# saninsteinn/django-assistant-bot

Measured on AMD Instinct MI355X. Metric: RAG queries/sec + p50 end-to-end latency, bge-base + Llama-3-8B, 1/2/4/8 MI355X, higher is better.
Workload: dtype bf16; 1 GPU; model=bge-base-en + llama-3-8b, global_batch=128, seq_len=1090, parallelism=dp1, mode=batch, index_rows=1000000, index=single shard, local top-k (no collective), sampling=temperature=1.0 top_k=50 top_p=0.95 ignore_eos, graphs=True

## Files before the change

django_assistant_bot_amd/build.py:

```python
from __future__ import annotations

import argparse
import concurrent.futures as cf
import os
import subprocess
import sys
import sysconfig
from pathlib import Path

PKG = Path(__file__).resolve().parent
CSRC = PKG / "csrc"
BUILD = PKG / "_build"
ARCH = os.environ.get("DAB_OFFLOAD_ARCH", "gfx950")


def _hipcc() -> str:
    rocm = os.environ.get("ROCM_PATH", "/opt/rocm")
    cand = Path(rocm) / "bin" / "hipcc"
    return str(cand) if cand.exists() else "hipcc"


def ext_path() -> Path:
    suffix = sysconfig.get_config_var("EXT_SUFFIX") or ".so"
    return PKG / f"_native{suffix}"
# ... 73 lines not shown
        raise RuntimeError(f"native build failed for: {failed}")
    if force or jobs_list or not out.exists():
        link = [hipcc, f"--offload-arch={ARCH}", "-shared", "-fPIC", *[str(o) for o in objs], "-o", str(out), "-lpthread", "-ldl"]
        cmd, rc, log = _compile(link)
        if rc:
            print(" ".join(cmd), file=sys.stderr)
            print(log, file=sys.stderr)
            raise RuntimeError("native link failed")
    return out


SANITIZERS = {"asan": ["-fsanitize=address,undefined", "-fno-omit-frame-pointer", "-fno-sanitize-recover=undefined"],
              "tsan": ["-fsanitize=thread"]}


def selftest(kind: str = "asan", out_dir: Path | None = None) -> tuple[int, str]:
    out_dir = out_dir or BUILD
    out_dir.mkdir(exist_ok=True)
    exe = out_dir / f"runtime_selftest_{kind}"
    srcs = [CSRC / "tests" / "runtime_selftest.cpp", *sorted((CSRC / "runtime").glob("*.cpp"))]
    cmd = ["g++", "-std=c++17", "-g", "-O1", *SANITIZERS[kind], f"-I{CSRC}", *map(str, srcs), "-o", str(exe),
           "-ldl", "-lpthread"]
    _, rc, log = _compile(cmd)
    if rc:
        return rc, log
    p = subprocess.run([str(exe)], stdout=subprocess.PIPE, stderr=subprocess.STDOUT, text=True, timeout=600)
    return p.returncode, p.stdout


def main() -> None:
    ap = argparse.ArgumentParser(description=__doc__)
    ap.add_argument("--force", action="store_true")
    ap.add_argument("-j", "--jobs", type=int, default=None)
    ap.add_argument("--debug", action="store_true")
    ap.add_argument("-v", "--verbose", action="store_true")
    ap.add_argument("--selftest", choices=sorted(SANITIZERS), default=None)
    a = ap.parse_args()
    if a.selftest:
        rc, log = selftest(a.selftest)
        print(log)
        sys.exit(rc)
    print(build(force=a.force, jobs=a.jobs, debug=a.debug, verbose=a.verbose))


if __name__ == "__main__":
    main()
```

django_assistant_bot_amd/csrc/bindings.cpp:

```cpp
#include <hip/hip_runtime.h>
#include <pybind11/numpy.h>
#include <pybind11/pybind11.h>
#include <pybind11/stl.h>

#include <stdexcept>
#include <string>

#include "kernels/launchers.h"
#include "runtime/json_grammar.h"
#include "runtime/kv_manager.h"
#include "runtime/rag.h"
#include "runtime/tokenizer.h"
#include "runtime/trace.h"

namespace py = pybind11;
using u = uintptr_t;

#define VP(x) reinterpret_cast<void*>(x)
#define CVP(x) reinterpret_cast<const void*>(x)
#define ST(x) reinterpret_cast<hipStream_t>(x)

static void check(int err, const char* name) {
  if (err) throw std::runtime_error(std::string("dab kernel '") + name + "' failed: " + hipGetErrorString((hipError_t)err));
}

PYBIND11_MODULE(_native, m) {
// ... 379 lines not shown
           [](dab::SchemaMatcher& j, int remaining, u out) {
             py::gil_scoped_release rel;
             return j.fill_mask(remaining, (uint32_t*)out);
           })
      .def("advance", &dab::SchemaMatcher::advance)
      .def("done", &dab::SchemaMatcher::done)
      .def("broken", &dab::SchemaMatcher::broken)
      .def("completion_len", &dab::SchemaMatcher::completion_len)
      .def("text", [](const dab::SchemaMatcher& j) { return py::bytes(j.text()); });
  m.def("json_accepts", [](const py::bytes& b, bool complete, int max_depth, int max_ws) {
    return dab::json_accepts(std::string(b), complete, max_depth, max_ws);
  }, py::arg("bytes"), py::arg("complete") = true, py::arg("max_depth") = 64, py::arg("max_ws") = 255);

  py::class_<dab::KVBlockManager>(m, "KVBlockManager")
      .def(py::init<int, int, bool>(), py::arg("num_blocks"), py::arg("block_size"), py::arg("prefix_cache") = true)
      .def("add_sequence", &dab::KVBlockManager::add_sequence)
      .def("extend", &dab::KVBlockManager::extend)
      .def("append_tokens", &dab::KVBlockManager::append_tokens)
      .def("commit_prefix", &dab::KVBlockManager::commit_prefix)
      .def("free_sequence", &dab::KVBlockManager::free_sequence)
      .def("has", &dab::KVBlockManager::has)
      .def("num_tokens", &dab::KVBlockManager::num_tokens)
      .def("capacity_tokens", &dab::KVBlockManager::capacity_tokens)
      .def("num_free_blocks", &dab::KVBlockManager::num_free_blocks)
      .def("num_blocks", &dab::KVBlockManager::num_blocks)
      .def("block_size", &dab::KVBlockManager::block_size)
      .def("prefix_hits", &dab::KVBlockManager::prefix_hits)
      .def("blocks", &dab::KVBlockManager::blocks)
      .def("slot_mapping_into",
           [](const dab::KVBlockManager& k, int64_t seq, int start, int n, u out) {
             k.slot_mapping(seq, start, n, (int64_t*)out);
// ... 36 lines not shown
```

django_assistant_bot_amd/csrc/runtime/kv_manager.cpp:

```cpp
#include "kv_manager.h"

#include <algorithm>
#include <functional>
#include <iterator>
#include <stdexcept>

namespace dab {

KVBlockManager::KVBlockManager(int num_blocks, int block_size, bool prefix_cache)
    : num_blocks_(num_blocks), block_size_(block_size), prefix_cache_(prefix_cache) {
  if (num_blocks <= 0 || block_size <= 0) throw std::invalid_argument("num_blocks and block_size must be > 0");
  free_.reserve(num_blocks);
  for (int b = 0; b < num_blocks; ++b) free_.push_back(b);
  lru_cap_ = std::max(64, num_blocks / 4);
  ref_.assign(num_blocks, 0);
  block_hash_.assign(num_blocks, 0);
  lru_pos_.resize(num_blocks);
  in_lru_.assign(num_blocks, 0);
}

uint64_t KVBlockManager::chain_hash(uint64_t parent, const int32_t* toks, int n) const {
  uint64_t h = parent ^ 0x9E3779B97F4A7C15ull;
  for (int i = 0; i < n; ++i) {
    h ^= (uint64_t)(uint32_t)toks[i] + 0x9E3779B97F4A7C15ull + (h << 6) + (h >> 2);
// ... 35 lines not shown
      block_hash_[e] = 0;
      push_free(e);
    }
  } else {
    block_hash_[b] = 0;
    push_free(b);
  }
}

void KVBlockManager::push_free(int32_t b) {
  free_.push_back(b);
  std::push_heap(free_.begin(), free_.end(), std::greater<int32_t>());
}

int KVBlockManager::add_sequence(int64_t seq_id, const std::vector<int32_t>& tokens, int reserve) {
  if (seqs_.count(seq_id)) throw std::invalid_argument("sequence already registered");
  const int n = (int)tokens.size();
  const int need_tokens = n + (reserve > 0 ? reserve : 0);
  const int need_blocks = (need_tokens + block_size_ - 1) / block_size_;
  std::vector<int32_t> hit_blocks;
  std::vector<uint64_t> hit_hashes;
  if (prefix_cache_ && n > 1) {
    const int max_full = (n - 1) / block_size_;
    uint64_t h = 0;
    for (int i = 0; i < max_full; ++i) {
      h = chain_hash(h, tokens.data() + (size_t)i * block_size_, block_size_);
      auto it = cached_.find(h);
      if (it == cached_.end()) break;
      hit_blocks.push_back(it->second);
      hit_hashes.push_back(h);
    }
  }
  int reused_from_lru = 0;
  for (int32_t b : hit_blocks) reused_from_lru += in_lru_[b] ? 1 : 0;
  const int fresh = need_blocks - (int)hit_blocks.size();
  if (fresh > num_free_blocks() - reused_from_lru) return -1;
  Seq s;
  for (int32_t b : hit_blocks) {
    if (in_lru_[b]) {
      lru_.erase(lru_pos_[b]);
      in_lru_[b] = 0;
    }
    ++ref_[b];
    s.blocks.push_back(b);
  }
  s.hashes = hit_hashes;
  for (int i = 0; i < fresh; ++i) s.blocks.push_back(alloc_block());
  s.tokens = tokens;
  const int cached_tokens = (int)hit_blocks.size() * block_size_;
  prefix_hits_ += cached_tokens;
  seqs_.emplace(seq_id, std::move(s));
  return cached_tokens;
}

bool KVBlockManager::extend(int64_t seq_id, int n) {
  auto it = seqs_.find(seq_id);
  if (it == seqs_.end()) throw std::invalid_argument("unknown sequence");
  Seq& s = it->second;
  const int need = (int)s.tokens.size() + n;
  const int need_blocks = (need + block_size_ - 1) / block_size_;
  const int more = need_blocks - (int)s.blocks.size();
  if (more <= 0) return true;
  if (more > num_free_blocks()) return false;
// ... 36 lines not shown

int KVBlockManager::num_tokens(int64_t seq_id) const {
  auto it = seqs_.find(seq_id);
  return it == seqs_.end() ? 0 : (int)it->second.tokens.size();
}

int KVBlockManager::capacity_tokens(int64_t seq_id) const {
  auto it = seqs_.find(seq_id);
  return it == seqs_.end() ? 0 : (int)it->second.blocks.size() * block_size_;
}

const std::vector<int32_t>& KVBlockManager::blocks(int64_t seq_id) const {
  auto it = seqs_.find(seq_id);
  if (it == seqs_.end()) throw std::invalid_argument("unknown sequence");
  return it->second.blocks;
}

void KVBlockManager::slot_mapping(int64_t seq_id, int start, int n, int64_t* out) const {
  const auto& bl = blocks(seq_id);
  for (int i = 0; i < n; ++i) {
    const int pos = start + i;
    const int bi = pos / block_size_;
    if (bi >= (int)bl.size()) throw std::out_of_range("slot beyond allocated blocks");
    out[i] = (int64_t)bl[bi] * block_size_ + (pos % block_size_);
  }
}

int KVBlockManager::prepare_decode(const std::vector<int64_t>& seq_ids, const std::vector<int32_t>& tokens,
                                   int max_blocks, int32_t* ids, int32_t* pos, int64_t* slots, int32_t* ctx,
                                   int32_t* block_table) {
// ... 34 lines not shown
```

django_assistant_bot_amd/csrc/runtime/kv_manager.h:

```cpp
#pragma once
#include <cstdint>
#include <list>
#include <unordered_map>
#include <vector>

namespace dab {

class KVBlockManager {
 public:
  KVBlockManager(int num_blocks, int block_size, bool prefix_cache);

  int add_sequence(int64_t seq_id, const std::vector<int32_t>& tokens, int reserve);
  bool extend(int64_t seq_id, int n);
  void append_tokens(int64_t seq_id, const std::vector<int32_t>& tokens);
  void commit_prefix(int64_t seq_id, int n_computed);
  void free_sequence(int64_t seq_id);

  bool has(int64_t seq_id) const { return seqs_.count(seq_id) != 0; }
  int num_tokens(int64_t seq_id) const;
  int capacity_tokens(int64_t seq_id) const;
  int num_free_blocks() const { return (int)free_.size() + (int)lru_.size(); }
  int num_blocks() const { return num_blocks_; }
  int block_size() const { return block_size_; }
  int64_t prefix_hits() const { return prefix_hits_; }
  const std::vector<int32_t>& blocks(int64_t seq_id) const;

  int prepare_decode(const std::vector<int64_t>& seq_ids, const std::vector<int32_t>& tokens, int max_blocks,
                     int32_t* ids, int32_t* pos, int64_t* slots, int32_t* ctx, int32_t* block_table);
  void slot_mapping(int64_t seq_id, int start, int n, int64_t* out) const;
  void block_table(const std::vector<int64_t>& seq_ids, int max_blocks, int32_t* out) const;

 private:
  struct Seq {
    std::vector<int32_t> blocks;
    std::vector<int32_t> tokens;
    std::vector<uint64_t> hashes;
  };
  int num_blocks_, block_size_;
  bool prefix_cache_;
  std::vector<int32_t> free_;
// ... 18 lines not shown
```

django_assistant_bot_amd/engine/llm_engine.py:

```python
from __future__ import annotations

import itertools
import math
import os
import time
from collections import deque
from dataclasses import dataclass, field

import numpy as np
import torch

from .. import ops
from ..models import AttnMeta, KVCache, LlamaModel, decoder_config, random_decoder_weights
from ..models.configs import DecoderConfig
from ..ops._lib import native
from ..utils import trace
from .tokenizer import Tokenizer


@dataclass
class SamplingParams:
    max_new_tokens: int = 1024
    temperature: float = 1.0
    top_k: int = 50
# ... 10 lines not shown

@dataclass
class GenerationOutput:
    request_id: int
    prompt_ids: list
    token_ids: list
    text: str
    finish_reason: str
    usage: dict
    timings: dict


@dataclass
class _Req:
    rid: int
    prompt: list
    params: SamplingParams
    arrival: float
    out: list = field(default_factory=list)
    computed: int = 0
    admitted: bool = False
    first_token_t: float = 0.0
    finish_t: float = 0.0
    finish_reason: str = ""
    rng_base: int = 0
    prefill_s: float = 0.0
    preempted: int = 0
    matcher: object = None

    @property
    def seq(self):
        return self.rid

    def full_prompt(self):
        return self.prompt + self.out if self.preempted else self.prompt




def _bucket_sizes(max_batch):
    b = [1, 2, 4, 8, 16, 24, 32, 48, 64, 96, 128, 160, 192, 224, 256, 320, 384, 448, 512]
    return [x for x in b if x < max_batch] + [max_batch]


class LLMEngine:
    def __init__(self, model: str | DecoderConfig = "llama-3-8b", device=None, weights: dict | None = None,
                 checkpoint: str | None = None, seed: int = 0, max_batch: int = 256, block_size: int = 64,
                 max_model_len: int | None = None, kv_cache_gb: float | None = None, num_blocks: int | None = None,
                 max_prefill_tokens: int = 16384, use_graphs: bool = True, prefix_cache: bool = True,
                 tp_group=None, tp_size: int = 1, tp_rank: int = 0, interleaved_mlp: bool = True,
                 part_size: int = 512, kv_memory_fraction: float = 0.85, mixed_prefill_tokens: int = 0,
                 pipeline_decode: bool = True, shared_model: LlamaModel | None = None,
                 kv_cache_dtype: str | None = None, kv_scratch_blocks: int | None = None,
                 weight_dtype: str | None = None):
        self.cfg = decoder_config(model) if isinstance(model, str) else model
        cfg = self.cfg
        if shared_model is not None:
            have = getattr(shared_model, "weight_dtype", "bf16")
            if weight_dtype is not None and weight_dtype != have:
                raise ValueError(f"weight_dtype={weight_dtype!r} conflicts with the shared model's {have!r}")
            weight_dtype = have
        elif weight_dtype is None:
            weight_dtype = os.environ.get("DAB_WEIGHT_DTYPE") or "bf16"
        if weight_dtype not in ("bf16", "fp8"):
            raise ValueError(f"weight_dtype must be 'bf16' or 'fp8', got {weight_dtype!r}")
        if weight_dtype == "fp8" and tp_size > 1:
            raise ValueError("weight_dtype='fp8' does not support tensor parallelism (tp_size > 1) yet")
        self.weight_dtype = weight_dtype
        if kv_cache_dtype is None:
# ... 100 lines not shown
        self._h_bt = mk((mb, self.max_blocks_per_seq), dtype=torch.int32)
        self._h_temp = mk(mb, dtype=torch.float32)
        self._h_topk = mk(mb, dtype=torch.int32)
        self._h_topp = mk(mb, dtype=torch.float32)
        self._h_cnt = mk(mb, dtype=torch.int64)
        self._h_tokens = mk(mb, dtype=torch.int32)
        self._h_order = mk(mb, dtype=torch.int32)
        self.pipeline_decode = bool(pipeline_decode) and tp_size == 1
        self._h_alt = {k: mk(*(getattr(self, k).shape,), dtype=getattr(self, k).dtype)
                       for k in ("_h_ids", "_h_pos", "_h_slots", "_h_ctx", "_h_bt", "_h_temp", "_h_topk", "_h_topp",
                                 "_h_cnt", "_h_tokens", "_h_order")}
        self._inflight = None
        self._d_mask = None
        self._masked = False
        self._pending_prefill = None
        max_parts = math.ceil(self.max_model_len / part_size)
        self._workspace = ops.DecodeWorkspace(mb, cfg.heads // tp_size, cfg.head_dim, max_parts, dev) if self.is_gpu \
            else None
        self._sample_ws = ops.kernels.sample_workspace(mb, cfg.vocab_size, dev) if self.is_gpu else None
        self.vp = bool(getattr(self.model, "vocab_parallel", False))
        self._vp_cand = None
        if self.vp and self.is_gpu:
            ncl = ops.kernels.sample_candidates_per_row(self.model.vocab_local)
            self._vp_cand = torch.zeros((2, mb, ncl), dtype=torch.int32, device=dev)
        self._graphs: dict = {}
        self._buckets = _bucket_sizes(max_batch)
        self._graph_pool = None
        self.timer = trace.GpuTimer(enabled=self.is_gpu)
        self.fault_hook = None
        self.auto_expire = True

    def add_request(self, prompt_ids: list, params: SamplingParams | None = None, request_id: int | None = None) -> int:
        params = params or SamplingParams()
        rid = next(self._ids) if request_id is None else request_id
        prompt = [int(t) for t in prompt_ids]
        if not prompt:
            prompt = [self.cfg.bos_id]
        if len(prompt) >= self.max_model_len:
            prompt = prompt[-(self.max_model_len - 1):]
        seed = params.seed if params.seed is not None else self.seed
        r = _Req(rid, prompt, params, time.perf_counter(), rng_base=((seed * 1000003 + rid) & 0xFFFFFFFF) << 20)
        r.matcher = self.check_params(params, matcher=True)
        if r.matcher is not None:
            self._ensure_mask_buffers()
        self.waiting.append(r)
        return rid

    def check_params(self, params: SamplingParams, matcher: bool = False):
        if params.json_schema is not None and self.tokenizer.byte_exact:
            from .json_schema import automaton_for, matcher_for

            if not matcher:
                automaton_for(self.tokenizer, self.cfg.eos_ids, params.json_schema)
                return None
            return matcher_for(self.tokenizer, self.cfg.eos_ids, params.json_schema)
        if params.json_mode or params.json_schema is not None:
# ... 19 lines not shown

    def generate(self, prompts: list, params: SamplingParams | list | None = None) -> list[GenerationOutput]:
        plist = params if isinstance(params, list) else [params or SamplingParams()] * len(prompts)
        rids = []
        for p, sp in zip(prompts, plist):
            ids = self.tokenizer.encode(p) if isinstance(p, str) else p
            rids.append(self.add_request(ids, sp))
        while self.has_unfinished():
            self.step()
        return [self.pop_output(r) for r in rids]

    def pop_output(self, rid: int) -> GenerationOutput:
        r = self.finished.pop(rid)
        n_out = len(r.out)
        return GenerationOutput(
            request_id=rid, prompt_ids=r.prompt, token_ids=list(r.out),
            text=self.tokenizer.decode(r.out), finish_reason=r.finish_reason,
            usage={"prompt_tokens": len(r.prompt), "completion_tokens": n_out, "total_tokens": len(r.prompt) + n_out},
            timings={"queue_s": max(0.0, r.first_token_t - r.arrival - r.prefill_s),
                     "ttft_s": r.first_token_t - r.arrival, "total_s": r.finish_t - r.arrival,
                     "decode_s": r.finish_t - r.first_token_t, "prefill_s": r.prefill_s},
        )

    def step(self) -> list[int]:
        done_before = set(self.finished)
        if self.fault_hook is not None:
            self.fault_hook(self)
        if self.auto_expire:
            self.expire_deadlines()
        if self._pending_prefill is not None:
            chunks = self._schedule_prefill() if not self.running or self.mixed_prefill_tokens <= 0 else []
            if chunks:
                prev, self._pending_prefill = self._pending_prefill, None
                self._run_prefill(chunks)
                self._finish_prefill(prev)
                return [k for k in self.finished if k not in done_before]
            self._finish_prefill(self._pending_prefill)
            self._pending_prefill = None
        if self._inflight is not None and not self._can_pipeline():
            self._finish_inflight()
        if self._can_pipeline():
            self._step_pipelined()
        elif self.running and self.mixed_prefill_tokens > 0 and (self.waiting or self.prefilling):
            batch = self._reserve_decode()
            chunks = self._schedule_prefill(self.mixed_prefill_tokens) if batch else self._schedule_prefill()
            if chunks and batch:
                self._run_mixed(batch, chunks)
            elif chunks:
                self._run_prefill(chunks)
            elif batch:
# ... 43 lines not shown
        return [r.rid for q in (self.waiting, self.prefilling, self.running) for r in q
                if r.params.timeout_s is not None and now - r.arrival > r.params.timeout_s]

    def expire_deadlines(self) -> list[int]:
        ids = self.expired()
        for rid in ids:
            self.abort(rid, "timeout")
        return ids

    def _schedule_prefill(self, budget: int | None = None):
        budget = self.max_prefill_tokens if budget is None else budget
        chunks = []
        for r in self.prefilling:
            if budget <= 0:
                break
            total = len(r.full_prompt())
            n = min(total - r.computed, budget)
            if n > 0:
                chunks.append((r, r.computed, n))
                self.blocks.commit_prefix(r.seq, r.computed + n)
                budget -= n
        while self.waiting and budget > 0 and len(self.running) + len(self.prefilling) < self.max_batch:
            r = self.waiting[0]
            toks = r.full_prompt()
            cached = self.blocks.add_sequence(r.seq, toks, 1)
            if cached < 0:
                if not self.running and not self.prefilling:
                    raise RuntimeError("KV cache too small for a single request")
                break
            self.waiting.popleft()
            r.admitted = True
            r.computed = cached
            self.prefilling.append(r)
            n = min(len(toks) - cached, budget)
            chunks.append((r, cached, n))
            self.blocks.commit_prefix(r.seq, cached + n)
            budget -= n
        return chunks

    def _build_block_tables(self, seqs, out_host):
        self.blocks.block_table_into(seqs, self.max_blocks_per_seq, out_host.data_ptr())

    def _kv_prefill_plan(self, bt, ctx, cu) -> dict:
        if not (self.kv.fp8 and self.is_gpu):
            return {}
        p = ops.kv_prefill_plan(bt, ctx, cu, self.block_size, self.kv.scratch_blocks, self.device)
        return {"kv_blocks": p.blocks, "kv_scratch_bt": p.scratch_bt, "kv_groups": p.groups}

    def _run_prefill(self, chunks):
        t0 = time.perf_counter()
        B = len(chunks)
        T = sum(n for _, _, n in chunks)
        ids = np.empty(T, dtype=np.int32)
        pos = np.empty(T, dtype=np.int32)
        slots = torch.empty(T, dtype=torch.int64)
        cu = np.zeros(B + 1, dtype=np.int32)
        ctx = np.empty(B, dtype=np.int32)
        o = 0
        for i, (r, s, n) in enumerate(chunks):
            toks = r.full_prompt()
            ids[o:o + n] = toks[s:s + n]
            pos[o:o + n] = np.arange(s, s + n, dtype=np.int32)
            self.blocks.slot_mapping_into(r.seq, s, n, slots.data_ptr() + 8 * o)
            o += n
            cu[i + 1] = o
            ctx[i] = s + n
        bt = torch.zeros((B, self.max_blocks_per_seq), dtype=torch.int32)
        self._build_block_tables([r.seq for r, _, _ in chunks], bt)
        to = self._h2d
        meta = AttnMeta(decode=False, positions=to(pos), slots=to(slots), block_tables=to(bt), ctx_lens=to(ctx),
                        cu_q=to(cu), max_q=max(n for _, _, n in chunks), **self._kv_prefill_plan(bt, ctx, cu))
        last_rows = [i for i, (r, s, n) in enumerate(chunks) if s + n == len(r.full_prompt())]
        if last_rows:
            sel = self._h2d(torch.as_tensor([int(cu[i + 1]) - 1 for i in last_rows], dtype=torch.int32))
        else:
            sel = torch.empty(0, dtype=torch.int32, device=self.device)
        with self.timer.phase("prefill"):
            hidden = self.model.forward(to(ids), meta, self.kv, out_rows=sel)
        self.stats["prefill_tokens"] += T
        self.stats["prefill_steps"] += 1
        reqs, toks = [], []
        if last_rows:
            logits = self.model.logits(hidden)
            reqs = [chunks[i][0] for i in last_rows]
            toks = self._sample(logits, reqs, to_host=not self.is_gpu)
        for r, s, n in chunks:
            r.computed = s + n
            self.blocks.commit_prefix(r.seq, s + n)
        pend = (chunks, reqs, toks, t0)
        self._tp_fault_enqueue()
        if self.is_gpu:
            self._pending_prefill = pend
        else:
            self._finish_prefill(pend)

    def _finish_prefill(self, pend):
        chunks, reqs, toks, t0 = pend
        if torch.is_tensor(toks):
            toks = toks.cpu().tolist()
            self._tp_fault_check()
        self._collect_gpu_times(block=bool(reqs))
        now = time.perf_counter()
        for r, s, n in chunks:
            r.prefill_s += now - t0
        if reqs:
            for r, t in zip(reqs, toks):
                self.blocks.commit_prefix(r.seq, len(r.full_prompt()))
                self.prefilling.remove(r)
                r.first_token_t = r.first_token_t or now
                r.preempted = 0
                self.running.append(r)
                self._accept_token(r, int(t), now)

    def _h2d(self, a):
        t = torch.as_tensor(a)
        if not self.is_gpu:
            return t
        return t.pin_memory().to(self.device, non_blocking=True)

    def _run_mixed(self, batch: list, chunks):
        t0 = time.perf_counter()
        dev = self.device
# ... 78 lines not shown
    def _ensure_mask_buffers(self) -> None:
        if getattr(self, "_d_mask", None) is not None:
            return
        W = -(-self.cfg.vocab_size // 32)
        mb = self.max_batch
        pin = self.is_gpu
        self._h_masks = [(torch.zeros((mb, W), dtype=torch.int32, pin_memory=pin),
                          torch.zeros(mb, dtype=torch.int32, pin_memory=pin)) for _ in range(2)]
        self._mask_events = [None, None]
        self._mask_turn = 0
        self._d_mask = torch.zeros((mb, W), dtype=torch.int32, device=self.device)
        self._d_mflag = torch.zeros(mb, dtype=torch.int32, device=self.device)

    def _budget(self, r: _Req) -> int:
        n, p = len(r.out), r.params
        left = min(p.max_new_tokens - n, self.max_model_len - len(r.prompt) - n)
        if p.max_length is not None:
            left = min(left, p.max_length - len(r.prompt) - n)
        return max(left, 1)

    def _fill_masks(self, reqs, n_rows: int) -> bool:
        if not any(r.matcher is not None for r in reqs):
            return False
        t = self._mask_turn
        self._mask_turn ^= 1
        if self._mask_events[t] is not None:
            self._mask_events[t].synchronize()
        h_mask, h_flag = self._h_masks[t]
        h_flag[:n_rows] = 0
        row_bytes = h_mask.shape[1] * 4
        base = h_mask.data_ptr()
        for i, r in enumerate(reqs):
            if r.matcher is not None:
# ... 12 lines not shown
        ops.mask_logits(logits, self._d_mask[:rows], self._d_mflag[:rows], vocab=getattr(m, "vocab_local", None),
                        word_offset=getattr(m, "vocab_start", 0) // 32)

    def _vp_merge(self, cand, temp, topk, topp, cnt, out=None):
        import torch.distributed as dist

        src = cand.contiguous()
        if dist.get_backend(self.tp_group) != "nccl":
            src = src.cpu()
        parts = [torch.empty_like(src) for _ in range(self.tp_size)]
        dist.all_gather(parts, src, group=self.tp_group)
        allc = torch.stack(parts, 2).to(self.device)
        allc = allc.reshape(2, allc.shape[1], -1).contiguous()
        return ops.sample_merge(allc, temp, topk, topp, self.seed, cnt, self.cfg.vocab_size, out=out)

    def _sample(self, logits, reqs, to_host: bool = True):
        n = len(reqs)
        if self._fill_masks(reqs, n):
            self._mask(logits, n)
        temps = torch.tensor([r.params.temperature if r.params.do_sample else 0.0 for r in reqs], dtype=torch.float32)
        topk = torch.tensor([r.params.top_k for r in reqs], dtype=torch.int32)
        topp = torch.tensor([r.params.top_p for r in reqs], dtype=torch.float32)
        cnt = torch.tensor([r.rng_base + len(r.out) for r in reqs], dtype=torch.int64)
        if self.is_gpu:
            fast = all((0 < r.params.top_k <= ops.kernels.SAMPLE_FAST_MAX_K) or not r.params.do_sample
                       or r.params.temperature <= 0 for r in reqs)
            h = self._h2d
            if self.vp and fast:
                cand = ops.sample_candidates(logits, self.model.vocab_local, self.model.vocab_start)
                toks = self._vp_merge(cand, h(temps), h(topk), h(topp), h(cnt))
            else:
                if self.vp:
                    logits = self.model.full_logits(logits)
                toks = ops.sample_tokens(logits, h(temps), h(topk), h(topp), self.seed, h(cnt), fast=fast)
                toks = self._tp_sync_tokens(toks)
            return toks.cpu().tolist() if to_host else toks
        if self.vp:
            logits = self.model.full_logits(logits)
        g = torch.Generator().manual_seed(int(self.seed * 7919 + int(cnt[0]) if n else 0))
        return ops.sample_tokens(logits, temps, topk, topp, self.seed, cnt, generator=g).tolist()

    def _tp_fault_enqueue(self) -> None:
# ... 18 lines not shown
        r.out.append(tok)
        p = r.params
        reason = ""
        json_done = False
        if r.matcher is not None:
            if r.matcher.advance(tok):
                json_done = r.matcher.done()
            else:
                self.stats["json_broken"] = self.stats.get("json_broken", 0) + 1
        if json_done:
            reason = "stop"
        elif not p.ignore_eos and (tok in self.cfg.eos_ids or tok in p.stop_token_ids):
            reason = "stop"
        elif len(r.out) >= p.max_new_tokens:
            reason = "length"
        elif p.max_length is not None and len(r.prompt) + len(r.out) >= p.max_length:
            reason = "length"
        elif len(r.prompt) + len(r.out) >= self.max_model_len:
            reason = "length"
        if reason:
            r.finish_reason = reason
            r.finish_t = now
            self.running.remove(r)
            self.blocks.free_sequence(r.seq)
            self.finished[r.rid] = r

    def _preempt_one(self, protect: _Req | None) -> bool:
        for victim in reversed(self.running):
            if victim is protect:
                continue
            self.running.remove(victim)
            self.blocks.free_sequence(victim.seq)
            victim.preempted = 1
# ... 3 lines not shown
            return True
        return False

    def _can_pipeline(self) -> bool:
        return bool(self.pipeline_decode and self.running and not self.waiting and not self.prefilling
                    and not any(r.matcher is not None for r in self.running))

    def _swap_host_buffers(self) -> None:
        for k, alt in self._h_alt.items():
            cur = getattr(self, k)
            setattr(self, k, alt)
            self._h_alt[k] = cur

    def _length_done(self, r: _Req, extra: int) -> bool:
        n, p = len(r.out) + extra, r.params
        return (n >= p.max_new_tokens or (p.max_length is not None and len(r.prompt) + n >= p.max_length)
                or len(r.prompt) + n >= self.max_model_len)

    def _step_pipelined(self):
        prev = self._inflight
        if prev is None:
            batch = self._reserve_decode()
            if not batch:
                return
            self._launch_decode(batch, None)
            prev = self._inflight
        nxt = [r for r in prev["batch"] if not r.finish_reason and not self._length_done(r, 1)]
        launched = False
        if nxt:
            self._swap_host_buffers()
            fail = self.blocks.prepare_decode_into(
                [r.seq for r in nxt], [r.out[-1] if r.out else 0 for r in nxt], self.max_blocks_per_seq,
# ... 230 lines not shown
```

django_assistant_bot_amd/engine/rag.py:

```python
from __future__ import annotations

import time
from dataclasses import dataclass, field
from datetime import datetime

import numpy as np

from ..ops._lib import native
from ..utils import trace
from .llm_engine import LLMEngine, SamplingParams


@dataclass
class StoredDocument:
    id: int
    name: str
    path: str
    content: str


@dataclass
class RAGResult:
    question: str
    answer: str
# ... 103 lines not shown
            out.append((docs_q, dbg))
        return out

    def build_prompts(self, questions: list[str], retrieved, now: datetime | None = None):
        prompts, used_docs = [], []
        for q, (docs_q, _) in zip(questions, retrieved):
            info, used = fill_info(docs_q, self.context_size, self.max_tokens_share, self.max_documents)
            messages = []
            if self.system_text:
                messages.append({"role": "system", "content": self.system_text})
            messages.append({"role": "user", "content": q})
            messages.append({"role": "system", "content": final_info_message(info, q, now)})
            prompts.append(render_messages(messages))
            used_docs.append(used)
        flat, offs = self.llm.tokenizer.encode_batch(prompts, add_special=True, max_len=self.llm.max_model_len - 1)
        flat, offs = np.asarray(flat), np.asarray(offs)
        token_lists = [flat[offs[i]:offs[i + 1]].tolist() for i in range(len(prompts))]
        return token_lists, used_docs

    def submit(self, questions: list[str], params: SamplingParams | None = None, bot_group: int | None = None,
               now: datetime | None = None) -> list[int]:
        params = params or SamplingParams(max_new_tokens=1024)
        t0 = time.perf_counter()
        if self._retrieve_lock is not None:
            with self._retrieve_lock:
                retrieved = self.retrieve(questions, bot_group)
                t_ret = time.perf_counter()
                token_lists, used_docs = self.build_prompts(questions, retrieved, now)
        else:
            retrieved = self.retrieve(questions, bot_group)
            t_ret = time.perf_counter()
            token_lists, used_docs = self.build_prompts(questions, retrieved, now)
        t_prompt = time.perf_counter()
# ... 37 lines not shown
```

Baseline: 40.15 queries/s.

## Plan prefill steps natively into double-buffered pinned staging with one H2D copy

Adds a C++ prefill step planner that writes token ids, positions, slot mappings, cu_q, context lengths, block tables and last-row indices straight into a pinned host staging arena. The arena is double-buffered and reaches the device with a single non-blocking copy, so the next step can be planned while the previous one is in flight. Prompts are now kept as int32 numpy views rather than Python lists, which removes per-token Python conversion in the RAG prompt path and the KV manager. The aim is to cut Python-side prefill preparation and the many small H2D transfers per step, at the cost of more code paths, event synchronisation and buffer-reuse hazards.

```diff
diff --git a/django_assistant_bot_amd/build.py b/django_assistant_bot_amd/build.py
--- a/django_assistant_bot_amd/build.py
+++ b/django_assistant_bot_amd/build.py
@@ -111,11 +111,16 @@
               "tsan": ["-fsanitize=thread"]}
 
 
-def selftest(kind: str = "asan", out_dir: Path | None = None) -> tuple[int, str]:
+SELFTESTS = ("runtime_selftest", "step_planner_selftest")
+
+
+def selftest(kind: str = "asan", out_dir: Path | None = None, name: str = "runtime_selftest") -> tuple[int, str]:
+    if name not in SELFTESTS:
+        raise ValueError(f"unknown selftest {name!r}: {SELFTESTS}")
     out_dir = out_dir or BUILD
     out_dir.mkdir(exist_ok=True)
-    exe = out_dir / f"runtime_selftest_{kind}"
-    srcs = [CSRC / "tests" / "runtime_selftest.cpp", *sorted((CSRC / "runtime").glob("*.cpp"))]
+    exe = out_dir / f"{name}_{kind}"
+    srcs = [CSRC / "tests" / f"{name}.cpp", *sorted((CSRC / "runtime").glob("*.cpp"))]
     cmd = ["g++", "-std=c++17", "-g", "-O1", *SANITIZERS[kind], f"-I{CSRC}", *map(str, srcs), "-o", str(exe),
            "-ldl", "-lpthread"]
     _, rc, log = _compile(cmd)
@@ -132,9 +137,10 @@
     ap.add_argument("--debug", action="store_true")
     ap.add_argument("-v", "--verbose", action="store_true")
     ap.add_argument("--selftest", choices=sorted(SANITIZERS), default=None)
+    ap.add_argument("--selftest-name", choices=SELFTESTS, default=SELFTESTS[0])
     a = ap.parse_args()
     if a.selftest:
-        rc, log = selftest(a.selftest)
+        rc, log = selftest(a.selftest, name=a.selftest_name)
         print(log)
         sys.exit(rc)
     print(build(force=a.force, jobs=a.jobs, debug=a.debug, verbose=a.verbose))
diff --git a/django_assistant_bot_amd/csrc/bindings.cpp b/django_assistant_bot_amd/csrc/bindings.cpp
--- a/django_assistant_bot_amd/csrc/bindings.cpp
+++ b/django_assistant_bot_amd/csrc/bindings.cpp
@@ -10,6 +10,7 @@
 #include "runtime/json_grammar.h"
 #include "runtime/kv_manager.h"
 #include "runtime/rag.h"
+#include "runtime/step_planner.h"
 #include "runtime/tokenizer.h"
 #include "runtime/trace.h"
 
@@ -419,7 +420,35 @@
 
   py::class_<dab::KVBlockManager>(m, "KVBlockManager")
       .def(py::init<int, int, bool>(), py::arg("num_blocks"), py::arg("block_size"), py::arg("prefix_cache") = true)
-      .def("add_sequence", &dab::KVBlockManager::add_sequence)
+      .def("add_sequence",
+           [](dab::KVBlockManager& k, int64_t seq, py::array_t<int32_t, py::array::c_style> toks, int reserve) {
+             if (toks.ndim() != 1) throw std::invalid_argument("tokens must be a 1-D int32 array");
+             return k.add_sequence(seq, toks.data(), (int)toks.shape(0), reserve);
+           })
+      .def("add_sequence", py::overload_cast<int64_t, const std::vector<int32_t>&, int>(&dab::KVBlockManager::add_sequence))
+      .def("tokens",
+           [](const dab::KVBlockManager& k, int64_t seq) {
+             const auto& t = k.tokens(seq);
+             py::array_t<int32_t> a(t.size());
+             std::copy(t.begin(), t.end(), a.mutable_data());
+             return a;
+           })
+      .def("plan_prefill_into",
+           [](const dab::KVBlockManager& k, const std::vector<std::tuple<int64_t, int32_t, int32_t>>& chunks, u ids,
+              u pos, u slots, u cu_q, u ctx_lens, u block_table, u row_width, u last_idx, u last_rows, int max_tokens,
+              int max_rows, int max_blocks) {
+             std::vector<dab::PrefillChunk> cs;
+             cs.reserve(chunks.size());
+             for (const auto& c : chunks) cs.push_back({std::get<0>(c), std::get<1>(c), std::get<2>(c)});
+             dab::PrefillPlanBuffers out{(int32_t*)ids, (int32_t*)pos, (int64_t*)slots, (int32_t*)cu_q,
+                                         (int32_t*)ctx_lens, (int32_t*)block_table, (int32_t*)row_width,
+                                         (int32_t*)last_idx, (int32_t*)last_rows, max_tokens, max_rows, max_blocks};
+             const auto info = dab::plan_prefill(k, cs.data(), (int)cs.size(), out);
+             return py::make_tuple(info.tokens, info.max_q, info.n_last);
+           },
+           py::arg("chunks"), py::arg("ids"), py::arg("pos"), py::arg("slots"), py::arg("cu_q"), py::arg("ctx_lens"),
+           py::arg("block_table"), py::arg("row_width"), py::arg("last_idx"), py::arg("last_rows"),
+           py::arg("max_tokens"), py::arg("max_rows"), py::arg("max_blocks"))
       .def("extend", &dab::KVBlockManager::extend)
       .def("append_tokens", &dab::KVBlockManager::append_tokens)
       .def("commit_prefix", &dab::KVBlockManager::commit_prefix)
diff --git a/django_assistant_bot_amd/csrc/runtime/kv_manager.cpp b/django_assistant_bot_amd/csrc/runtime/kv_manager.cpp
--- a/django_assistant_bot_amd/csrc/runtime/kv_manager.cpp
+++ b/django_assistant_bot_amd/csrc/runtime/kv_manager.cpp
@@ -73,8 +73,12 @@
 }
 
 int KVBlockManager::add_sequence(int64_t seq_id, const std::vector<int32_t>& tokens, int reserve) {
+  return add_sequence(seq_id, tokens.data(), (int)tokens.size(), reserve);
+}
+
+int KVBlockManager::add_sequence(int64_t seq_id, const int32_t* tokens, int n, int reserve) {
   if (seqs_.count(seq_id)) throw std::invalid_argument("sequence already registered");
-  const int n = (int)tokens.size();
+  if (n < 0 || (n > 0 && tokens == nullptr)) throw std::invalid_argument("bad token array");
   const int need_tokens = n + (reserve > 0 ? reserve : 0);
   const int need_blocks = (need_tokens + block_size_ - 1) / block_size_;
   std::vector<int32_t> hit_blocks;
@@ -83,7 +87,7 @@
     const int max_full = (n - 1) / block_size_;
     uint64_t h = 0;
     for (int i = 0; i < max_full; ++i) {
-      h = chain_hash(h, tokens.data() + (size_t)i * block_size_, block_size_);
+      h = chain_hash(h, tokens + (size_t)i * block_size_, block_size_);
       auto it = cached_.find(h);
       if (it == cached_.end()) break;
       hit_blocks.push_back(it->second);
@@ -105,7 +109,7 @@
   }
   s.hashes = hit_hashes;
   for (int i = 0; i < fresh; ++i) s.blocks.push_back(alloc_block());
-  s.tokens = tokens;
+  s.tokens.assign(tokens, tokens + n);
   const int cached_tokens = (int)hit_blocks.size() * block_size_;
   prefix_hits_ += cached_tokens;
   seqs_.emplace(seq_id, std::move(s));
@@ -172,6 +176,12 @@
   auto it = seqs_.find(seq_id);
   if (it == seqs_.end()) throw std::invalid_argument("unknown sequence");
   return it->second.blocks;
+}
+
+const std::vector<int32_t>& KVBlockManager::tokens(int64_t seq_id) const {
+  auto it = seqs_.find(seq_id);
+  if (it == seqs_.end()) throw std::invalid_argument("unknown sequence");
+  return it->second.tokens;
 }
 
 void KVBlockManager::slot_mapping(int64_t seq_id, int start, int n, int64_t* out) const {
diff --git a/django_assistant_bot_amd/csrc/runtime/kv_manager.h b/django_assistant_bot_amd/csrc/runtime/kv_manager.h
--- a/django_assistant_bot_amd/csrc/runtime/kv_manager.h
+++ b/django_assistant_bot_amd/csrc/runtime/kv_manager.h
@@ -11,6 +11,7 @@
   KVBlockManager(int num_blocks, int block_size, bool prefix_cache);
 
   int add_sequence(int64_t seq_id, const std::vector<int32_t>& tokens, int reserve);
+  int add_sequence(int64_t seq_id, const int32_t* tokens, int n, int reserve);
   bool extend(int64_t seq_id, int n);
   void append_tokens(int64_t seq_id, const std::vector<int32_t>& tokens);
   void commit_prefix(int64_t seq_id, int n_computed);
@@ -24,6 +25,7 @@
   int block_size() const { return block_size_; }
   int64_t prefix_hits() const { return prefix_hits_; }
   const std::vector<int32_t>& blocks(int64_t seq_id) const;
+  const std::vector<int32_t>& tokens(int64_t seq_id) const;
 
   int prepare_decode(const std::vector<int64_t>& seq_ids, const std::vector<int32_t>& tokens, int max_blocks,
                      int32_t* ids, int32_t* pos, int64_t* slots, int32_t* ctx, int32_t* block_table);
diff --git a/django_assistant_bot_amd/csrc/runtime/step_planner.cpp b/django_assistant_bot_amd/csrc/runtime/step_planner.cpp
--- /dev/null
+++ b/django_assistant_bot_amd/csrc/runtime/step_planner.cpp
@@ -0,0 +1,63 @@
+#include "step_planner.h"
+
+#include <algorithm>
+#include <stdexcept>
+#include <string>
+
+namespace dab {
+
+PrefillPlanInfo plan_prefill(const KVBlockManager& kv, const PrefillChunk* chunks, int n_chunks,
+                             const PrefillPlanBuffers& out) {
+  if (n_chunks <= 0) throw std::invalid_argument("a prefill step needs at least one chunk");
+  if (n_chunks > out.max_rows)
+    throw std::out_of_range("prefill step of " + std::to_string(n_chunks) + " chunks exceeds the staging rows (" +
+                            std::to_string(out.max_rows) + ")");
+  const int bs = kv.block_size();
+  int64_t total = 0;
+  for (int i = 0; i < n_chunks; ++i) {
+    const PrefillChunk& c = chunks[i];
+    if (c.n <= 0 || c.start < 0) throw std::invalid_argument("prefill chunk with n <= 0 or start < 0");
+    const int have = (int)kv.tokens(c.seq).size();
+    const int64_t end = (int64_t)c.start + c.n;
+    if (end > have) throw std::out_of_range("prefill chunk past the end of its prompt");
+    const auto& bl = kv.blocks(c.seq);
+    if ((int)bl.size() > out.max_blocks) throw std::out_of_range("block table wider than max_blocks");
+    if ((end + bs - 1) / bs > (int64_t)bl.size()) throw std::out_of_range("slot beyond allocated blocks");
+    total += c.n;
+  }
+  if (total > out.max_tokens)
+    throw std::out_of_range("prefill step of " + std::to_string(total) + " tokens exceeds the staging tokens (" +
+                            std::to_string(out.max_tokens) + ")");
+  PrefillPlanInfo info{0, 0, 0};
+  int o = 0;
+  out.cu_q[0] = 0;
+  for (int i = 0; i < n_chunks; ++i) {
+    const PrefillChunk& c = chunks[i];
+    const auto& toks = kv.tokens(c.seq);
+    const auto& bl = kv.blocks(c.seq);
+    std::copy(toks.begin() + c.start, toks.begin() + c.start + c.n, out.ids + o);
+    for (int j = 0; j < c.n; ++j) {
+      const int p = c.start + j;
+      out.pos[o + j] = p;
+      out.slots[o + j] = (int64_t)bl[p / bs] * bs + (p % bs);
+    }
+    o += c.n;
+    out.cu_q[i + 1] = o;
+    out.ctx_lens[i] = c.start + c.n;
+    int32_t* row = out.block_table + (size_t)i * out.max_blocks;
+    const int w = (int)bl.size();
+    std::copy(bl.begin(), bl.end(), row);
+    if (out.row_width[i] > w) std::fill(row + w, row + out.row_width[i], 0);
+    out.row_width[i] = w;
+    info.max_q = std::max(info.max_q, (int)c.n);
+    if (c.start + c.n == (int)toks.size()) {
+      out.last_idx[info.n_last] = i;
+      out.last_rows[info.n_last] = o - 1;
+      ++info.n_last;
+    }
+  }
+  info.tokens = o;
+  return info;
+}
+
+}
diff --git a/django_assistant_bot_amd/csrc/runtime/step_planner.h b/django_assistant_bot_amd/csrc/runtime/step_planner.h
--- /dev/null
+++ b/django_assistant_bot_amd/csrc/runtime/step_planner.h
@@ -0,0 +1,38 @@
+#pragma once
+#include <cstdint>
+
+#include "kv_manager.h"
+
+namespace dab {
+
+struct PrefillChunk {
+  int64_t seq;
+  int32_t start;
+  int32_t n;
+};
+
+struct PrefillPlanBuffers {
+  int32_t* ids;
+  int32_t* pos;
+  int64_t* slots;
+  int32_t* cu_q;
+  int32_t* ctx_lens;
+  int32_t* block_table;
+  int32_t* row_width;
+  int32_t* last_idx;
+  int32_t* last_rows;
+  int max_tokens;
+  int max_rows;
+  int max_blocks;
+};
+
+struct PrefillPlanInfo {
+  int tokens;
+  int max_q;
+  int n_last;
+};
+
+PrefillPlanInfo plan_prefill(const KVBlockManager& kv, const PrefillChunk* chunks, int n_chunks,
+                             const PrefillPlanBuffers& out);
+
+}
diff --git a/django_assistant_bot_amd/engine/llm_engine.py b/django_assistant_bot_amd/engine/llm_engine.py
--- a/django_assistant_bot_amd/engine/llm_engine.py
+++ b/django_assistant_bot_amd/engine/llm_engine.py
@@ -48,9 +48,11 @@
 @dataclass
 class _Req:
     rid: int
-    prompt: list
+    prompt_np: np.ndarray
     params: SamplingParams
     arrival: float
+    prompt_len: int = 0
+    prompt_list: list | None = None
     out: list = field(default_factory=list)
     computed: int = 0
     admitted: bool = False
@@ -66,9 +68,26 @@
     def seq(self):
         return self.rid
 
+    @property
+    def prompt(self) -> list:
+        if self.prompt_list is None:
+            self.prompt_list = self.prompt_np.tolist()
+        return self.prompt_list
+
     def full_prompt(self):
         return self.prompt + self.out if self.preempted else self.prompt
 
+    def full_prompt_np(self) -> np.ndarray:
+        if self.preempted and self.out:
+            return np.concatenate([self.prompt_np, np.asarray(self.out, dtype=np.int32)])
+        return self.prompt_np
+
+    def full_len(self) -> int:
+        return self.prompt_len + len(self.out) if self.preempted else self.prompt_len
+
+
+def _planner_enabled() -> bool:
+    return os.environ.get("DAB_STEP_PLANNER", "1").strip().lower() not in ("0", "false", "off", "no")
 
 
 
@@ -86,7 +105,7 @@
                  part_size: int = 512, kv_memory_fraction: float = 0.85, mixed_prefill_tokens: int = 0,
                  pipeline_decode: bool = True, shared_model: LlamaModel | None = None,
                  kv_cache_dtype: str | None = None, kv_scratch_blocks: int | None = None,
-                 weight_dtype: str | None = None):
+                 weight_dtype: str | None = None, step_planner: bool | None = None):
         self.cfg = decoder_config(model) if isinstance(model, str) else model
         cfg = self.cfg
         if shared_model is not None:
@@ -217,6 +236,12 @@
         self._d_mask = None
         self._masked = False
         self._pending_prefill = None
+        self.step_planner = _planner_enabled() if step_planner is None else bool(step_planner)
+        self._staging = None
+        if self.step_planner:
+            from .step_planner import PrefillStaging
+
+            self._staging = PrefillStaging(max_prefill_tokens, mb, self.max_blocks_per_seq, dev)
         max_parts = math.ceil(self.max_model_len / part_size)
         self._workspace = ops.DecodeWorkspace(mb, cfg.heads // tp_size, cfg.head_dim, max_parts, dev) if self.is_gpu \
             else None
@@ -236,13 +261,22 @@
     def add_request(self, prompt_ids: list, params: SamplingParams | None = None, request_id: int | None = None) -> int:
         params = params or SamplingParams()
         rid = next(self._ids) if request_id is None else request_id
-        prompt = [int(t) for t in prompt_ids]
-        if not prompt:
-            prompt = [self.cfg.bos_id]
+        plist = None
+        if isinstance(prompt_ids, np.ndarray) and prompt_ids.dtype == np.int32 and prompt_ids.ndim == 1:
+            prompt = prompt_ids
+            if not len(prompt):
+                prompt = np.asarray([self.cfg.bos_id], dtype=np.int32)
+        else:
+            plist = [int(t) for t in prompt_ids] or [self.cfg.bos_id]
+            if len(plist) >= self.max_model_len:
+                plist = plist[-(self.max_model_len - 1):]
+            prompt = np.asarray(plist, dtype=np.int32)
         if len(prompt) >= self.max_model_len:
             prompt = prompt[-(self.max_model_len - 1):]
+        prompt = np.ascontiguousarray(prompt)
         seed = params.seed if params.seed is not None else self.seed
-        r = _Req(rid, prompt, params, time.perf_counter(), rng_base=((seed * 1000003 + rid) & 0xFFFFFFFF) << 20)
+        r = _Req(rid, prompt, params, time.perf_counter(), prompt_len=len(prompt), prompt_list=plist,
+                 rng_base=((seed * 1000003 + rid) & 0xFFFFFFFF) << 20)
         r.matcher = self.check_params(params, matcher=True)
         if r.matcher is not None:
             self._ensure_mask_buffers()
@@ -292,9 +326,9 @@
         r = self.finished.pop(rid)
         n_out = len(r.out)
         return GenerationOutput(
-            request_id=rid, prompt_ids=r.prompt, token_ids=list(r.out),
+            request_id=rid, prompt_ids=r.prompt_np if r.prompt_list is None else r.prompt_list, token_ids=list(r.out),
             text=self.tokenizer.decode(r.out), finish_reason=r.finish_reason,
-            usage={"prompt_tokens": len(r.prompt), "completion_tokens": n_out, "total_tokens": len(r.prompt) + n_out},
+            usage={"prompt_tokens": r.prompt_len, "completion_tokens": n_out, "total_tokens": r.prompt_len + n_out},
             timings={"queue_s": max(0.0, r.first_token_t - r.arrival - r.prefill_s),
                      "ttft_s": r.first_token_t - r.arrival, "total_s": r.finish_t - r.arrival,
                      "decode_s": r.finish_t - r.first_token_t, "prefill_s": r.prefill_s},
@@ -311,7 +345,7 @@
             if chunks:
                 prev, self._pending_prefill = self._pending_prefill, None
                 self._run_prefill(chunks)
-                self._finish_prefill(prev)
+                self._finish_prefill(prev, next_in_flight=True)
                 return [k for k in self.finished if k not in done_before]
             self._finish_prefill(self._pending_prefill)
             self._pending_prefill = None
@@ -385,7 +419,7 @@
         for r in self.prefilling:
             if budget <= 0:
                 break
-            total = len(r.full_prompt())
+            total = r.full_len()
             n = min(total - r.computed, budget)
             if n > 0:
                 chunks.append((r, r.computed, n))
@@ -393,7 +427,7 @@
                 budget -= n
         while self.waiting and budget > 0 and len(self.running) + len(self.prefilling) < self.max_batch:
             r = self.waiting[0]
-            toks = r.full_prompt()
+            toks = r.full_prompt_np()
             cached = self.blocks.add_sequence(r.seq, toks, 1)
             if cached < 0:
                 if not self.running and not self.prefilling:
@@ -420,6 +454,47 @@
 
     def _run_prefill(self, chunks):
         t0 = time.perf_counter()
+        plan = None
+        if self._staging is not None:
+            ids_d, meta, sel, last_rows, staged, plan = self._plan_prefill_native(chunks)
+        else:
+            ids_d, meta, sel, last_rows, staged = self._plan_prefill_python(chunks)
+        T = sum(n for _, _, n in chunks)
+        with self.timer.phase("prefill"):
+            hidden = self.model.forward(ids_d, meta, self.kv, out_rows=sel)
+        self.stats["prefill_tokens"] += T
+        self.stats["prefill_steps"] += 1
+        reqs, toks = [], []
+        if last_rows:
+            logits = self.model.logits(hidden)
+            reqs = [chunks[i][0] for i in last_rows]
+            toks = self._sample(logits, reqs, to_host=not self.is_gpu, staged=staged)
+        for r, s, n in chunks:
+            r.computed = s + n
+            self.blocks.commit_prefix(r.seq, s + n)
+        self._tp_fault_enqueue()
+        if plan is not None and torch.is_tensor(toks) and toks.is_cuda:
+            toks = self._staging.read_back(plan, toks)
+        pend = (chunks, reqs, toks, t0)
+        if self.is_gpu:
+            self._pending_prefill = pend
+        else:
+            self._finish_prefill(pend)
+
+    def _sampling_params(self, reqs):
+        return ([r.params.temperature if r.params.do_sample else 0.0 for r in reqs], [r.params.top_k for r in reqs],
+                [r.params.top_p for r in reqs], [r.rng_base + len(r.out) for r in reqs])
+
+    def _plan_prefill_native(self, chunks):
+        p = self._staging.plan(self.blocks, [(r.seq, s, n) for r, s, n in chunks],
+                               lambda idx: self._sampling_params([chunks[i][0] for i in idx]))
+        meta = AttnMeta(decode=False, positions=p.pos, slots=p.slots, block_tables=p.block_tables,
+                        ctx_lens=p.ctx_lens, cu_q=p.cu_q, max_q=p.max_q,
+                        **self._kv_prefill_plan(p.h_block_tables, p.h_ctx_lens, p.h_cu_q))
+        staged = (p.temp, p.top_k, p.top_p, p.counters) if self.is_gpu else None
+        return p.ids, meta, p.last_rows, p.last_idx, staged, p
+
+    def _plan_prefill_python(self, chunks):
         B = len(chunks)
         T = sum(n for _, _, n in chunks)
         ids = np.empty(T, dtype=np.int32)
@@ -446,37 +521,25 @@
             sel = self._h2d(torch.as_tensor([int(cu[i + 1]) - 1 for i in last_rows], dtype=torch.int32))
         else:
             sel = torch.empty(0, dtype=torch.int32, device=self.device)
-        with self.timer.phase("prefill"):
-            hidden = self.model.forward(to(ids), meta, self.kv, out_rows=sel)
-        self.stats["prefill_tokens"] += T
-        self.stats["prefill_steps"] += 1
-        reqs, toks = [], []
-        if last_rows:
-            logits = self.model.logits(hidden)
-            reqs = [chunks[i][0] for i in last_rows]
-            toks = self._sample(logits, reqs, to_host=not self.is_gpu)
-        for r, s, n in chunks:
-            r.computed = s + n
-            self.blocks.commit_prefix(r.seq, s + n)
-        pend = (chunks, reqs, toks, t0)
-        self._tp_fault_enqueue()
-        if self.is_gpu:
-            self._pending_prefill = pend
-        else:
-            self._finish_prefill(pend)
-
-    def _finish_prefill(self, pend):
+        return to(ids), meta, sel, last_rows, None
+
+    def _finish_prefill(self, pend, next_in_flight: bool = False):
         chunks, reqs, toks, t0 = pend
+        waits_for_next = True
         if torch.is_tensor(toks):
             toks = toks.cpu().tolist()
             self._tp_fault_check()
-        self._collect_gpu_times(block=bool(reqs))
+        elif hasattr(toks, "tokens"):
+            toks = toks.tokens()
+            self._tp_fault_check()
+            waits_for_next = False
+        self._collect_gpu_times(block=bool(reqs) and (waits_for_next or not next_in_flight))
         now = time.perf_counter()
         for r, s, n in chunks:
             r.prefill_s += now - t0
         if reqs:
             for r, t in zip(reqs, toks):
-                self.blocks.commit_prefix(r.seq, len(r.full_prompt()))
+                self.blocks.commit_prefix(r.seq, r.full_len())
                 self.prefilling.remove(r)
                 r.first_token_t = r.first_token_t or now
                 r.preempted = 0
@@ -585,9 +648,9 @@
 
     def _budget(self, r: _Req) -> int:
         n, p = len(r.out), r.params
-        left = min(p.max_new_tokens - n, self.max_model_len - len(r.prompt) - n)
+        left = min(p.max_new_tokens - n, self.max_model_len - r.prompt_len - n)
         if p.max_length is not None:
-            left = min(left, p.max_length - len(r.prompt) - n)
+            left = min(left, p.max_length - r.prompt_len - n)
         return max(left, 1)
 
     def _fill_masks(self, reqs, n_rows: int) -> bool:
@@ -630,18 +693,22 @@
         allc = allc.reshape(2, allc.shape[1], -1).contiguous()
         return ops.sample_merge(allc, temp, topk, topp, self.seed, cnt, self.cfg.vocab_size, out=out)
 
-    def _sample(self, logits, reqs, to_host: bool = True):
+    def _sample(self, logits, reqs, to_host: bool = True, staged=None):
         n = len(reqs)
         if self._fill_masks(reqs, n):
             self._mask(logits, n)
-        temps = torch.tensor([r.params.temperature if r.params.do_sample else 0.0 for r in reqs], dtype=torch.float32)
-        topk = torch.tensor([r.params.top_k for r in reqs], dtype=torch.int32)
-        topp = torch.tensor([r.params.top_p for r in reqs], dtype=torch.float32)
-        cnt = torch.tensor([r.rng_base + len(r.out) for r in reqs], dtype=torch.int64)
+        if staged is not None and self.is_gpu:
+            temps, topk, topp, cnt = staged
+        else:
+            temps = torch.tensor([r.params.temperature if r.params.do_sample else 0.0 for r in reqs],
+                                 dtype=torch.float32)
+            topk = torch.tensor([r.params.top_k for r in reqs], dtype=torch.int32)
+            topp = torch.tensor([r.params.top_p for r in reqs], dtype=torch.float32)
+            cnt = torch.tensor([r.rng_base + len(r.out) for r in reqs], dtype=torch.int64)
         if self.is_gpu:
             fast = all((0 < r.params.top_k <= ops.kernels.SAMPLE_FAST_MAX_K) or not r.params.do_sample
                        or r.params.temperature <= 0 for r in reqs)
-            h = self._h2d
+            h = self._h2d if staged is None else (lambda t: t)
             if self.vp and fast:
                 cand = ops.sample_candidates(logits, self.model.vocab_local, self.model.vocab_start)
                 toks = self._vp_merge(cand, h(temps), h(topk), h(topp), h(cnt))
@@ -690,9 +757,9 @@
             reason = "stop"
         elif len(r.out) >= p.max_new_tokens:
             reason = "length"
-        elif p.max_length is not None and len(r.prompt) + len(r.out) >= p.max_length:
+        elif p.max_length is not None and r.prompt_len + len(r.out) >= p.max_length:
             reason = "length"
-        elif len(r.prompt) + len(r.out) >= self.max_model_len:
+        elif r.prompt_len + len(r.out) >= self.max_model_len:
             reason = "length"
         if reason:
             r.finish_reason = reason
@@ -726,8 +793,8 @@
 
     def _length_done(self, r: _Req, extra: int) -> bool:
         n, p = len(r.out) + extra, r.params
-        return (n >= p.max_new_tokens or (p.max_length is not None and len(r.prompt) + n >= p.max_length)
-                or len(r.prompt) + n >= self.max_model_len)
+        return (n >= p.max_new_tokens or (p.max_length is not None and r.prompt_len + n >= p.max_length)
+                or r.prompt_len + n >= self.max_model_len)
 
     def _step_pipelined(self):
         prev = self._inflight
diff --git a/django_assistant_bot_amd/engine/rag.py b/django_assistant_bot_amd/engine/rag.py
--- a/django_assistant_bot_amd/engine/rag.py
+++ b/django_assistant_bot_amd/engine/rag.py
@@ -141,9 +141,10 @@
             prompts.append(render_messages(messages))
             used_docs.append(used)
         flat, offs = self.llm.tokenizer.encode_batch(prompts, add_special=True, max_len=self.llm.max_model_len - 1)
-        flat, offs = np.asarray(flat), np.asarray(offs)
-        token_lists = [flat[offs[i]:offs[i + 1]].tolist() for i in range(len(prompts))]
-        return token_lists, used_docs
+        flat = np.ascontiguousarray(flat, dtype=np.int32)
+        offs = np.asarray(offs).tolist()
+        token_views = [flat[offs[i]:offs[i + 1]] for i in range(len(prompts))]
+        return token_views, used_docs
 
     def submit(self, questions: list[str], params: SamplingParams | None = None, bot_group: int | None = None,
                now: datetime | None = None) -> list[int]:
diff --git a/django_assistant_bot_amd/engine/step_planner.py b/django_assistant_bot_amd/engine/step_planner.py
--- /dev/null
+++ b/django_assistant_bot_amd/engine/step_planner.py
@@ -0,0 +1,131 @@
+from __future__ import annotations
+
+from dataclasses import dataclass
+
+import numpy as np
+import torch
+
+_ALIGN = 256
+
+
+def _up(n: int) -> int:
+    return -(-n // _ALIGN) * _ALIGN
+
+
+@dataclass
+class PrefillPlan:
+    tokens: int
+    max_q: int
+    last_idx: list
+    ids: torch.Tensor
+    pos: torch.Tensor
+    slots: torch.Tensor
+    cu_q: torch.Tensor
+    ctx_lens: torch.Tensor
+    block_tables: torch.Tensor
+    last_rows: torch.Tensor
+    temp: torch.Tensor
+    top_k: torch.Tensor
+    top_p: torch.Tensor
+    counters: torch.Tensor
+    h_block_tables: torch.Tensor
+    h_ctx_lens: np.ndarray
+    h_cu_q: np.ndarray
+    staging_set: object = None
+
+
+class PrefillReadBack:
+
+    def __init__(self, host: torch.Tensor, event):
+        self.host, self.event = host, event
+
+    def tokens(self) -> list:
+        self.event.synchronize()
+        return self.host.tolist()
+
+
+class _Set:
+    def __init__(self, nbytes: int, head: dict, mb: int, max_blocks: int, device: torch.device):
+        gpu = device.type == "cuda"
+        self.host = torch.zeros(nbytes, dtype=torch.uint8, pin_memory=gpu)
+        self.dev = torch.zeros(nbytes, dtype=torch.uint8, device=device) if gpu else self.host
+        self.event = torch.cuda.Event() if gpu else None
+        self.read_event = torch.cuda.Event() if gpu else None
+        self.in_flight = False
+        self.row_width = np.zeros(mb, dtype=np.int32)
+        self.h, self.d = {}, {}
+        for name, (off, count, dtype) in head.items():
+            nb = count * torch.empty(0, dtype=dtype).element_size()
+            self.h[name] = self.host[off:off + nb].view(dtype)
+            self.d[name] = self.dev[off:off + nb].view(dtype)
+        self.h["bt"] = self.h["bt"].view(mb, max_blocks)
+        self.d["bt"] = self.d["bt"].view(mb, max_blocks)
+
+
+class PrefillStaging:
+    def __init__(self, max_tokens: int, max_batch: int, max_blocks: int, device, n_sets: int = 2):
+        if n_sets < 2:
+            raise ValueError("the engine keeps one prefill step in flight while it plans the next: n_sets >= 2")
+        self.max_tokens, self.max_batch, self.max_blocks = int(max_tokens), int(max_batch), int(max_blocks)
+        self.device = torch.device(device)
+        mb = self.max_batch
+        sections = (("cu", mb + 1, torch.int32), ("ctx", mb, torch.int32), ("sel", mb, torch.int32),
+                    ("idx", mb, torch.int32), ("tok", mb, torch.int32), ("temp", mb, torch.float32), ("topk", mb, torch.int32),
+                    ("topp", mb, torch.float32), ("cnt", mb, torch.int64), ("bt", mb * self.max_blocks, torch.int32))
+        self._head, off = {}, 0
+        for name, count, dtype in sections:
+            self._head[name] = (off, count, dtype)
+            off = _up(off + count * torch.empty(0, dtype=dtype).element_size())
+        self._tail = off
+        nbytes = self._tail + _up(8 * self.max_tokens) + 2 * _up(4 * self.max_tokens)
+        self.sets = [_Set(nbytes, self._head, mb, self.max_blocks, self.device) for _ in range(n_sets)]
+        self._turn = 0
+        self.steps = 0
+
+    def plan(self, blocks, chunks, sampling=None) -> PrefillPlan:
+        st = self.sets[self._turn]
+        self._turn = (self._turn + 1) % len(self.sets)
+        self.steps += 1
+        if st.in_flight:
+            st.event.synchronize()
+            st.in_flight = False
+        T = sum(c[2] for c in chunks)
+        B = len(chunks)
+        o_slots = self._tail
+        o_ids = o_slots + _up(8 * T)
+        o_pos = o_ids + _up(4 * T)
+        end = o_pos + 4 * T
+        base = st.host.data_ptr()
+        h = st.h
+        tokens, max_q, n_last = blocks.plan_prefill_into(
+            chunks, base + o_ids, base + o_pos, base + o_slots, h["cu"].data_ptr(), h["ctx"].data_ptr(),
+            h["bt"].data_ptr(), st.row_width.ctypes.data, h["idx"].data_ptr(), h["sel"].data_ptr(),
+            self.max_tokens, self.max_batch, self.max_blocks)
+        assert tokens == T
+        last_idx = h["idx"][:n_last].tolist()
+        if n_last and sampling is not None:
+            temp, topk, topp, cnt = sampling(last_idx)
+            h["temp"][:n_last] = torch.tensor(temp, dtype=torch.float32)
+            h["topk"][:n_last] = torch.tensor(topk, dtype=torch.int32)
+            h["topp"][:n_last] = torch.tensor(topp, dtype=torch.float32)
+            h["cnt"][:n_last] = torch.tensor(cnt, dtype=torch.int64)
+        if st.event is not None:
+            st.dev[:end].copy_(st.host[:end], non_blocking=True)
+            st.event.record()
+            st.in_flight = True
+        d, dev = st.d, st.dev
+        return PrefillPlan(
+            tokens=T, max_q=max_q, last_idx=last_idx,
+            ids=dev[o_ids:o_ids + 4 * T].view(torch.int32), pos=dev[o_pos:o_pos + 4 * T].view(torch.int32),
+            slots=dev[o_slots:o_slots + 8 * T].view(torch.int64), cu_q=d["cu"][:B + 1], ctx_lens=d["ctx"][:B],
+            block_tables=d["bt"][:B], last_rows=d["sel"][:n_last], temp=d["temp"][:n_last], top_k=d["topk"][:n_last],
+            top_p=d["topp"][:n_last], counters=d["cnt"][:n_last], h_block_tables=h["bt"][:B],
+            h_ctx_lens=h["ctx"][:B].numpy(), h_cu_q=h["cu"][:B + 1].numpy(), staging_set=st)
+
+    @staticmethod
+    def read_back(plan: PrefillPlan, tokens: torch.Tensor) -> PrefillReadBack:
+        st = plan.staging_set
+        host = st.h["tok"][:tokens.numel()]
+        host.copy_(tokens, non_blocking=True)
+        st.read_event.record()
+        return PrefillReadBack(host, st.read_event)
```

Result: no change. 40.28 queries/s, median of 6 (+0.3%).
